# eboigne/PyTV-4D

Measured on NVIDIA B200. Metric: cp_iter_voxel_updates_per_s, higher is better.
Workload: dtype f32

## Files before the change

### pytv-4d_b200/csrc/adj_core.cuh

```cuda
#pragma once
#include "strip_core.cuh"

#ifndef PYTVB_STRIP_R
#define PYTVB_STRIP_R 4
#endif
#ifndef PYTVB_ADJ_R
#define PYTVB_ADJ_R 32
#endif

namespace pytvb {

constexpr int ADJ_R = PYTVB_ADJ_R;
constexpr int ADJ_MAXM = 8;
constexpr int ADJ_THREADS = 256;
static_assert(ADJ_R % PYTVB_STRIP_R == 0, "the L21 partial sums follow the row groups of cp_dual_strip_kernel");

PYTVB_HD int adj_tile_quads(int M) { return M == 1 ? 256 : (M == 2 ? 128 : (M <= 4 ? 64 : 32)); }

PYTVB_HD bool adj_edge_row(int i, int Ni) { return (i % ADJ_R == 0 && i > 0) || (i % ADJ_R == ADJ_R - 1 && i < Ni - 1); }
PYTVB_HD bool adj_edge_col(int tq, int TWq, int j0, int vec, int Nj) { return (tq == 0 && j0 > 0) || (tq == TWq - 1 && j0 + vec < Nj); }

template <int VEC> struct AdjSlots { static constexpr int value = 3 + 2 * VEC; };
template <typename T, int VEC>
struct AdjShared {
    T* b;
    PYTVB_HD T& jf0(int k) const { return b[k]; }
    PYTVB_HD T& jf1(int k) const { return b[ADJ_THREADS + k]; }
    PYTVB_HD T& jb0(int k) const { return b[2 * ADJ_THREADS + k]; }
    PYTVB_HD T& tf(int e, int k) const { return b[(3 + e) * ADJ_THREADS + k]; }
    PYTVB_HD T& tb(int e, int k) const { return b[(3 + VEC + e) * ADJ_THREADS + k]; }
};

template <typename T, int VEC, int SCHEME, bool Z_ON, bool T_ON>
struct AdjThread {
    static constexpr int ND = Comp<SCHEME, Z_ON, T_ON>::ND;
    DualPlane<T, T> pl;
    MirrorPlanes<T> mir;
    T* qp;
    int t, tq, j0, TWq;
    bool act, cedge;
    T at, bt;
    T yv[ND][VEC], tsc[VEC];
    T cIFm[VEC], cIF[VEC], cIB[VEC], cCol[VEC], cT[VEC];
    T g;
    double l21;
};

template <typename T, int VEC, int SCHEME, bool Z_ON, bool T_ON, bool MIR>
PYTVB_HD void adj_thread_init(AdjThread<T, VEC, SCHEME, Z_ON, T_ON>& s, const ImgView<T>& Xb, T* y, T* qd, const Params<T>& P, const MirrorBufs<T>& mb,
                              int z, int cb, int tid, int TWq, int W) {
    s.TWq = TWq;
    s.t = tid / TWq;
    s.tq = tid - s.t * TWq;
    const int qj = cb * TWq + s.tq;
    s.j0 = qj * VEC;
    s.act = s.t < P.M && qj < W;
    const int tc = s.t < P.M ? s.t : P.M - 1;
    s.pl = make_dual_plane<T, SCHEME, T>(Xb, y, P, z, tc);
    s.mir = MirrorPlanes<T>{nullptr, nullptr};
    if constexpr (MIR) s.mir = mirror_planes<T>(mb, P, z, tc);
    s.qp = qd + (long long)z * P.sZ + (long long)tc * P.sT;
    s.cedge = adj_edge_col(s.tq, TWq, s.j0, VEC, P.Nj);
    s.at = s.bt = T(0);
    if (T_ON) {
        adj_factors<T, SCHEME>(s.at, s.bt, tc, P.M, P.t_fwd_fallback != 0);
        s.at *= P.srt;
        s.bt *= P.srt;
    }
#pragma unroll
    for (int e = 0; e < VEC; ++e) s.cIFm[e] = s.cIF[e] = s.cIB[e] = s.cCol[e] = s.cT[e] = T(0);
    s.g = T(0);
    s.l21 = 0.0;
}

template <typename T, int VEC, int SCHEME, bool Z_ON, bool T_ON>
PYTVB_HD void adj_finish_row(AdjThread<T, VEC, SCHEME, Z_ON, T_ON>& s, const Params<T>& P, int k, const T* ib_next) {
    constexpr bool NF = (SCHEME != DOWNWIND), NB = (SCHEME != UPWIND), CTR = (SCHEME == CENTRAL);
    T a, b;
    adj_factors<T, SCHEME>(a, b, k, P.Ni, false);
    Pack<T, VEC> pk;
#pragma unroll
    for (int e = 0; e < VEC; ++e) {
        const T f_m = NF ? (k > 0 ? s.cIFm[e] : s.cIF[e]) : T(0);
        const T f_c = (!CTR && NF) ? s.cIF[e] : T(0);
        const T b_c = (!CTR && NB) ? s.cIB[e] : T(0);
        const T b_p = NB ? ib_next[e] : T(0);
        const T rows = adj_term<T, SCHEME>(a, b, f_m, f_c, b_c, b_p, false);
        pk.v[e] = s.cedge ? adj_rows_t<T, T_ON>(rows, s.cT[e]) : adj_prefix<T, T_ON>(rows, s.cCol[e], s.cT[e]);
    }
    if (!adj_edge_row(k, P.Ni)) st_pack<T, VEC>(s.qp + k * P.Nj + s.j0, pk);
}

template <typename T, int VEC, int SCHEME, bool Z_ON, bool T_ON>
PYTVB_HD void adj_prefetch_next(const AdjThread<T, VEC, SCHEME, Z_ON, T_ON>& s, const Params<T>& P, int i) {
#if defined(__CUDA_ARCH__)
    const int Nj = P.Nj, o = i * Nj + s.j0;
#pragma unroll
    for (int k = 0; k < Comp<SCHEME, Z_ON, T_ON>::ND; ++k) asm volatile("prefetch.global.L2 [%0];" ::"l"(s.pl.y + (long long)k * P.sC + o + Nj));
    asm volatile("prefetch.global.L2 [%0];" ::"l"(s.pl.c + (i + 2 < P.Ni ? o + 2 * Nj : o + Nj)));
#else
    (void)s; (void)P; (void)i;
#endif
}

template <typename T, int VEC, int SCHEME, bool Z_ON, bool T_ON, bool TS, bool MIR>
PYTVB_HD void adj_row_update(AdjThread<T, VEC, SCHEME, Z_ON, T_ON>& s, const Params<T>& P, int i, const AdjShared<T, VEC>& sh, int tid, T sig, T lam) {
    typedef Comp<SCHEME, Z_ON, T_ON> C;
    if (!s.act) return;
    const int Nj = P.Nj, o = i * Nj + s.j0;
    s.g += strip_quad_cp_dual_y<T, VEC, SCHEME, Z_ON, T_ON, T, TS, MIR>(s.yv, s.pl, P, i, s.j0, o, i > 0 ? o - Nj : o, i < P.Ni - 1 ? o + Nj : o, sig,
                                                                       lam, s.mir);
    if (i % PYTVB_STRIP_R == PYTVB_STRIP_R - 1 || i == P.Ni - 1) {
        s.l21 += (double)s.g * (double)P.inv_div;
        s.g = T(0);
    }
    sh.jf0(tid) = s.yv[C::J_F][0];
    sh.jf1(tid) = s.yv[C::J_F][VEC - 1];
    sh.jb0(tid) = s.yv[C::J_B][0];
    if (T_ON) {
#pragma unroll
        for (int e = 0; e < VEC; ++e) s.tsc[e] = T(1);
        if constexpr (TS) {
            const Pack<T, VEC> sc = ld_pack<T, VEC>(s.pl.ts + o);
#pragma unroll
            for (int e = 0; e < VEC; ++e) s.tsc[e] = sc.v[e];
        }
#pragma unroll
        for (int e = 0; e < VEC; ++e) {
            sh.tf(e, tid) = TS ? mul_rn(s.yv[C::T_F][e], s.tsc[e]) : s.yv[C::T_F][e];
            sh.tb(e, tid) = TS ? mul_rn(s.yv[C::T_B][e], s.tsc[e]) : s.yv[C::T_B][e];
        }
    }
}

template <typename T, int VEC, int SCHEME, bool Z_ON, bool T_ON, bool TS>
PYTVB_HD void adj_row_finish(AdjThread<T, VEC, SCHEME, Z_ON, T_ON>& s, const Params<T>& P, int i, bool first, const AdjShared<T, VEC>& sh, int tid) {
    typedef Comp<SCHEME, Z_ON, T_ON> C;
    constexpr bool NF = (SCHEME != DOWNWIND), NB = (SCHEME != UPWIND), CTR = (SCHEME == CENTRAL);
    constexpr bool HB = (SCHEME == HYBRID || SCHEME == DOWNWIND);
    if (!s.act) return;
    const int Nj = P.Nj, TWq = s.TWq;
    T col[VEC], tt[VEC];
    {
        T jb[VEC];
#pragma unroll
        for (int e = 0; e < VEC; ++e) jb[e] = (SCHEME == HYBRID) ? s.yv[C::J_B][e] : T(0);
        const bool has_l = s.j0 > 0 && s.tq > 0, has_r = s.j0 + VEC < Nj && s.tq < TWq - 1;
        const T jf_l = (NF && has_l) ? sh.jf1(tid - 1) : T(0);
        const T jf_r = (CTR && has_r) ? sh.jf0(tid + 1) : T(0);
        const T jb_r = (HB && has_r) ? sh.jb0(tid + 1) : T(0);
        adj_cols<T, VEC, SCHEME>(col, s.yv[C::J_F], jb, jf_l, jf_r, jb_r, s.j0, Nj);
    }
    if (T_ON) {
        const bool tfb = P.t_fwd_fallback != 0, up_form = !CTR || tfb;
        T ifs[VEC], f_m[VEC], f_c[VEC], b_c[VEC], b_p[VEC], fac[VEC];
#pragma unroll
        for (int e = 0; e < VEC; ++e) {
            ifs[e] = TS ? mul_rn(s.yv[C::I_F][e], s.tsc[e]) : s.yv[C::I_F][e];
            f_m[e] = NF ? (s.t > 0 ? sh.tf(e, tid - TWq) : ifs[e]) : T(0);
            f_c[e] = (up_form && NF) ? sh.tf(e, tid) : T(0);
            b_c[e] = (!CTR && NB) ? sh.tb(e, tid) : T(0);
            b_p[e] = (NB && !(CTR && tfb)) ? (s.t < P.M - 1 ? sh.tb(e, tid + TWq) : ifs[e]) : T(0);
        }
        static_factor<T, VEC>(fac, P, i, s.j0);
        adj_time<T, VEC, SCHEME>(tt, f_m, f_c, b_c, b_p, fac, s.at, s.bt, tfb);
    } else {
        zero_into<T, VEC>(tt);
    }
    if (!first) adj_finish_row(s, P, i - 1, s.yv[C::I_B]);
#pragma unroll
    for (int e = 0; e < VEC; ++e) {
        s.cIFm[e] = s.cIF[e];
        s.cIF[e] = s.yv[C::I_F][e];
        s.cIB[e] = s.yv[C::I_B][e];
        s.cCol[e] = col[e];
        s.cT[e] = tt[e];
    }
}

template <typename T, int VEC, int SCHEME, bool Z_ON, bool T_ON>
PYTVB_HD void adj_tile_end(AdjThread<T, VEC, SCHEME, Z_ON, T_ON>& s, const Params<T>& P, int i_end) {
    if (s.act && i_end == P.Ni) adj_finish_row(s, P, P.Ni - 1, s.cIB);
}

template <typename T, int VEC, int SCHEME, bool Z_ON, bool T_ON, int VARIANT, bool WM, bool TS, bool MIR>
PYTVB_HD T adj_quad_primal(const PrimalPlane<T, T>& pl, const T* qd, T* x, T* xbar, const T* x0, const T* w, const Params<T>& P, int i, int j0,
                           bool cedge, T tau, T c1, T theta, T tau_x0, MirrorPlanes<T> mir) {
    typedef Comp<SCHEME, Z_ON, T_ON> C;
    constexpr bool NF = (SCHEME != DOWNWIND), CTR = (SCHEME == CENTRAL), HB = (SCHEME == HYBRID || SCHEME == DOWNWIND);
    const int o = i * P.Nj + j0;
    T dty[VEC];
    if (adj_edge_row(i, P.Ni)) {
        strip_quad_DT<T, VEC, SCHEME, Z_ON, T_ON, false, T, TS>(dty, pl, P, i, j0, o, i > 0 ? o - P.Nj : o, i < P.Ni - 1 ? o + P.Nj : o);
    } else {
        const T* qo = qd + pl.img + o;
        const T* yJ_F = pl.y + (long long)C::J_F * P.sC + o;
        const T* yJ_B = pl.y + (long long)C::J_B * P.sC + o;
        const bool l = cedge && NF && j0 > 0, rf = cedge && CTR && j0 + VEC < P.Nj, rb = cedge && HB && j0 + VEC < P.Nj;
        T jf[VEC], jb[VEC];
        ld_into<T, VEC>(jf, cedge ? yJ_F : qo);
        if (SCHEME == HYBRID) ld_into<T, VEC>(jb, cedge ? yJ_B : qo); else zero_into<T, VEC>(jb);
        T jf_l = *(l ? yJ_F - 1 : qo), jf_r = *(rf ? yJ_F + VEC : qo), jb_r = *(rb ? yJ_B + VEC : qo);
        jf_l = l ? jf_l : T(0); jf_r = rf ? jf_r : T(0); jb_r = rb ? jb_r : T(0);
        const Pack<T, VEC> pre = ld_pack<T, VEC>(qo);
        T zt[VEC], cols[VEC];
        if (Z_ON) strip_quad_DT_z<T, VEC, SCHEME, Z_ON, T_ON, false, T>(zt, pl, P, o); else zero_into<T, VEC>(zt);
        adj_cols<T, VEC, SCHEME>(cols, jf, jb, jf_l, jf_r, jb_r, j0, P.Nj);
#pragma unroll
        for (int e = 0; e < VEC; ++e) dty[e] = adj_finish<T, Z_ON>(cedge ? add_rn(pre.v[e], cols[e]) : pre.v[e], zt[e], P.inv_div);
    }
    return cp_primal_update<T, VEC, Z_ON, VARIANT, MIR, WM>(dty, x, xbar, x0, pl.img + o, o, tau, c1, theta, tau_x0, mir, w);
}

}
```

### pytv-4d_b200/csrc/cp_adj.cu

```cuda
#include <stdlib.h>

#include "host_common.cuh"
#include "kernels2.cuh"
#include "adj_core.cuh"

using namespace pytvb;

namespace pytvb {

static_assert(ADJ_THREADS == CTA_THREADS, "an A' tile is one CTA");

struct AdjTiling {
    int TWq, W, ncb, nz;
    FastDiv d_ncb, d_nz;
    long long nblocks;
};
inline AdjTiling make_adj_tiling(int Nj, int Ni, int M, int nz, int vec) {
    AdjTiling t;
    t.TWq = adj_tile_quads(M);
    t.W = (Nj + vec - 1) / vec;
    t.ncb = (t.W + t.TWq - 1) / t.TWq;
    t.nz = nz;
    t.d_ncb = make_fastdiv((unsigned)t.ncb);
    t.d_nz = make_fastdiv((unsigned)nz);
    t.nblocks = (long long)t.ncb * nz * ((Ni + ADJ_R - 1) / ADJ_R);
    return t;
}

template <typename T, int VEC, int SCHEME, bool Z_ON, bool T_ON, bool TS, bool MIR>
__global__ void __launch_bounds__(CTA_THREADS, PYTVB_DUAL_MINB) cp_dual_adj_kernel(ImgView<T> Xb, T* __restrict__ y, T* __restrict__ qd,
                                                                                  double* __restrict__ partial, Params<T> P, T sig, T lam,
                                                                                  AdjTiling tl, MirrorBufs<T> mb) {
    __shared__ T sm[2][AdjSlots<T_ON ? VEC : 0>::value * CTA_THREADS];
    unsigned b = blockIdx.x, cb, zi;
    tl.d_ncb.divmod(b, b, cb);
    tl.d_nz.divmod(b, b, zi);
    const int i0 = (int)b * ADJ_R, nrows = min(ADJ_R, P.Ni - i0), tid = threadIdx.x;
    AdjThread<T, VEC, SCHEME, Z_ON, T_ON> s;
    adj_thread_init<T, VEC, SCHEME, Z_ON, T_ON, MIR>(s, Xb, y, qd, P, mb, (int)zi, (int)cb, tid, tl.TWq, tl.W);
    for (int r = 0; r < nrows; ++r) {
        const int bf = r & 1;
        const AdjShared<T, VEC> sh{sm[bf]};
        if (s.act && r + 1 < nrows) adj_prefetch_next(s, P, i0 + r);
        adj_row_update<T, VEC, SCHEME, Z_ON, T_ON, TS, MIR>(s, P, i0 + r, sh, tid, sig, lam);
        __syncthreads();
        adj_row_finish<T, VEC, SCHEME, Z_ON, T_ON, TS>(s, P, i0 + r, r == 0, sh, tid);
    }
    adj_tile_end(s, P, i0 + nrows);
    if (partial) {
        const double bs = block_sum(s.l21);
        store_or_finish(bs, partial, P);
    }
}

template <typename T, int VEC, int SCHEME, bool Z_ON, bool T_ON, int VARIANT, bool WM, int R, bool TS, bool MIR>
__global__ void __launch_bounds__(CTA_THREADS, PYTVB_PRIMAL_MINB) cp_primal_adj_kernel(FieldView<T> Y, const T* __restrict__ qd, T* __restrict__ x,
                                                                                      T* __restrict__ xbar, const T* __restrict__ x0,
                                                                                      const T* __restrict__ w, double* __restrict__ partial,
                                                                                      Params<T> P, T tau, T c1, T theta, T tau_x0, Tiling tl,
                                                                                      int twq, MirrorBufs<T> mb) {
    const QuadIdx q = decode_quad(tl, (P.Ni + R - 1) / R, VEC);
    T fid = T(0);
    if (q.active) {
        const PrimalPlane<T, T> pl = make_primal_plane<T, SCHEME, Z_ON, T_ON, T>(Y, P, q.z, q.t);
        MirrorPlanes<T> mir{nullptr, nullptr};
        if constexpr (MIR) mir = mirror_planes<T>(mb, P, q.z, q.t);
        const bool cedge = adj_edge_col((q.j0 / VEC) & (twq - 1), twq, q.j0, VEC, P.Nj);
        const int i0 = q.i * R;
#pragma unroll
        for (int r = 0; r < R; ++r) {
            const int i = i0 + r;
            if (i < P.Ni)
                fid += adj_quad_primal<T, VEC, SCHEME, Z_ON, T_ON, VARIANT, WM, TS, MIR>(pl, qd, x, xbar, x0, w, P, i, q.j0, cedge, tau, c1, theta, tau_x0,
                                                                                         mir);
        }
    }
    if (partial) {
        const double bs = block_sum((double)fid);
        store_or_finish(bs, partial, P);
    }
}

}

namespace {

template <typename T> struct AdjDualArgs { ImgView<T> Xb; T* y; T* q; double* partial; Params<T> P; T sig, lam; cudaStream_t st; long long* nb; T* mir_prev; T* mir_next; };

template <typename T, int VEC, int SCHEME, bool Z, bool TT> struct LaunchDualAdj {
    static int run(const AdjDualArgs<T>& a) {
        const AdjTiling tl = make_adj_tiling(a.P.Nj, a.P.Ni, a.P.M, a.P.Nz, VEC);
        PYTVB_REQUIRE(tl.nblocks > 0 && tl.nblocks < 2147483647LL, "grid of %lld CTAs is out of range", tl.nblocks);
        const bool ts = TT && a.P.tscale, mir = Z && (a.mir_prev || a.mir_next);
        const MirrorBufs<T> mb{a.mir_prev, a.mir_next};
        const unsigned nb = (unsigned)tl.nblocks;
        if (ts && mir) cp_dual_adj_kernel<T, VEC, SCHEME, Z, TT, TT, Z><<<nb, CTA_THREADS, 0, a.st>>>(a.Xb, a.y, a.q, a.partial, a.P, a.sig, a.lam, tl, mb);
        else if (ts) cp_dual_adj_kernel<T, VEC, SCHEME, Z, TT, TT, false><<<nb, CTA_THREADS, 0, a.st>>>(a.Xb, a.y, a.q, a.partial, a.P, a.sig, a.lam, tl, mb);
        else if (mir) cp_dual_adj_kernel<T, VEC, SCHEME, Z, TT, false, Z><<<nb, CTA_THREADS, 0, a.st>>>(a.Xb, a.y, a.q, a.partial, a.P, a.sig, a.lam, tl, mb);
        else cp_dual_adj_kernel<T, VEC, SCHEME, Z, TT, false, false><<<nb, CTA_THREADS, 0, a.st>>>(a.Xb, a.y, a.q, a.partial, a.P, a.sig, a.lam, tl, mb);
        count_launches(1);
        PYTVB_CUDA(cudaGetLastError());
        *a.nb = tl.nblocks;
        return PYTVB_OK;
    }
};

template <typename T> struct AdjPrimalArgs {
    FieldView<T> Y; const T* q; T* x; T* xbar; const T* x0; const T* w; double* partial; Params<T> P; T tau, theta; int term; cudaStream_t st;
    long long* nb; T* mir_prev; T* mir_next;
};

template <typename T, int VEC, int SCHEME, bool Z, bool TT, int VARIANT, bool WM>
void launch_primal_adj(const AdjPrimalArgs<T>& a, const Tiling& tl) {
    constexpr int R = PYTVB_STRIP_R;
    const bool ts = TT && a.P.tscale, mir = Z && (a.mir_prev || a.mir_next);
    const MirrorBufs<T> mb{a.mir_prev, a.mir_next};
    const unsigned nb = (unsigned)tl.nblocks;
    const T c1 = VARIANT == 0 ? T(1) / (T(1) + a.tau) : T(0), tx = VARIANT == 0 ? T(-1) : a.tau;
    const int twq = adj_tile_quads(a.P.M);
#define PYTVB_ADJ_B(TSV, MIRV)                                                                                                                  \
    cp_primal_adj_kernel<T, VEC, SCHEME, Z, TT, VARIANT, WM, R, TSV, MIRV><<<nb, CTA_THREADS, 0, a.st>>>(a.Y, a.q, a.x, a.xbar, a.x0, a.w, a.partial, \
                                                                                                      a.P, a.tau, c1, a.theta, tx, tl, twq, mb)
    if (ts && mir) PYTVB_ADJ_B(TT, Z);
    else if (ts) PYTVB_ADJ_B(TT, false);
    else if (mir) PYTVB_ADJ_B(false, Z);
    else PYTVB_ADJ_B(false, false);
#undef PYTVB_ADJ_B
}

template <typename T, int VEC, int SCHEME, bool Z, bool TT> struct LaunchPrimalAdj {
    static int run(const AdjPrimalArgs<T>& a) {
        const Tiling tl = make_strip_tiling<PYTVB_STRIP_R>(a.P.Nj, a.P.Ni, a.P.M, a.P.Nz, VEC);
        if (int rc = check_grid(tl)) return rc;
        if (a.term == PYTVB_DATA_L2 && !a.w) launch_primal_adj<T, VEC, SCHEME, Z, TT, 0, false>(a, tl);
        else if (a.term == PYTVB_DATA_L2) launch_primal_adj<T, VEC, SCHEME, Z, TT, 2, true>(a, tl);
        else if (a.w) launch_primal_adj<T, VEC, SCHEME, Z, TT, 3, true>(a, tl);
        else launch_primal_adj<T, VEC, SCHEME, Z, TT, 3, false>(a, tl);
        count_launches(1);
        PYTVB_CUDA(cudaGetLastError());
        *a.nb = tl.nblocks;
        return PYTVB_OK;
    }
};

template <typename T>
int run_dual_adj(const pytvb_problem* pb, const void* xbar, void* y, void* q, double lam, double sigma, double* d_l21, const void* lo, const void* hi,
                 void* mir_prev, void* mir_next, void* ws, cudaStream_t st) {
    const Axes ax = axes_of(pb);
    AdjDualArgs<T> a;
    a.Xb = ImgView<T>{(const T*)xbar, (const T*)lo, (const T*)hi, 1};
    a.y = (T*)y;
    a.q = (T*)q;
    a.partial = d_l21 ? reduce_partials(ws) : nullptr;
    a.P = make_params<T>(pb);
    arm_reduction(a.P, ws, d_l21);
    a.sig = (T)sigma * a.P.inv_div;
    a.lam = (T)lam;
    a.mir_prev = (T*)mir_prev; a.mir_next = (T*)mir_next;
    a.st = st;
    long long nb = 0;
    a.nb = &nb;
    const int vec = pick_vec<T>(pb, {xbar, y, q, lo, hi, mir_prev, mir_next});
    if (int rc = dispatch<LaunchDualAdj, T>(vec, pb->scheme, ax.z_on, ax.t_on, a)) return rc;
    return d_l21 ? finish_reduction(a.partial, nb, d_l21, st) : PYTVB_OK;
}

template <typename T>
int run_primal_adj(const pytvb_problem* pb, int term, const void* w, const void* y, const void* q, void* x, void* xbar, const void* x0, double tau,
                   double theta, double* d_fid, const void* lo, const void* hi, void* mir_prev, void* mir_next, void* ws, cudaStream_t st) {
    const Axes ax = axes_of(pb);
    AdjPrimalArgs<T> a;
    a.Y = FieldView<T>{(const T*)y, (const T*)lo, (const T*)hi};
    a.q = (const T*)q;
    a.x = (T*)x; a.xbar = (T*)xbar; a.x0 = (const T*)x0; a.w = (const T*)w;
    a.partial = d_fid ? reduce_partials(ws) : nullptr;
    a.P = make_params<T>(pb);
    arm_reduction(a.P, ws, d_fid);
    a.tau = (T)tau; a.theta = (T)theta;
    a.term = term;
    a.mir_prev = (T*)mir_prev; a.mir_next = (T*)mir_next;
    a.st = st;
    long long nb = 0;
    a.nb = &nb;
    const int vec = pick_vec<T>(pb, {y, q, x, xbar, x0, w, lo, hi, mir_prev, mir_next});
    if (int rc = dispatch<LaunchPrimalAdj, T>(vec, pb->scheme, ax.z_on, ax.t_on, a)) return rc;
    return d_fid ? finish_reduction(a.partial, nb, d_fid, st) : PYTVB_OK;
}

}

extern "C" {

int pytvb_cp_dual_adj_p2p(const pytvb_problem* pb, const void* xbar, void* y, void* q, double lam, double sigma, double* d_l21_or_null,
                          const void* halo_lo, const void* halo_hi, void* mirror_prev, void* mirror_next, void* ws, void* stream) {
    if (int rc = check_problem(pb)) return rc;
    PYTVB_REQUIRE(xbar && y && q, "xbar, y and q must not be NULL");
    PYTVB_REQUIRE(pb->M <= ADJ_MAXM, "M = %lld: the dual pass with the adjoint prefix spans at most %d frames", (long long)pb->M, ADJ_MAXM);
    PYTVB_REQUIRE(!d_l21_or_null || ws, "a reduction workspace is required when d_l21 is requested");
    PYTVB_REQUIRE(lam >= 0, "lam must be >= 0");
    if (int rc = check_halos(pb, axes_of(pb).z_on, false, halo_lo, halo_hi)) return rc;
    cudaStream_t st = (cudaStream_t)stream;
    return pb->dtype == PYTVB_F32 ? run_dual_adj<float>(pb, xbar, y, q, lam, sigma, d_l21_or_null, halo_lo, halo_hi, mirror_prev, mirror_next, ws, st)
                                  : run_dual_adj<double>(pb, xbar, y, q, lam, sigma, d_l21_or_null, halo_lo, halo_hi, mirror_prev, mirror_next, ws, st);
}

int pytvb_cp_dual_adj(const pytvb_problem* pb, const void* xbar, void* y, void* q, double lam, double sigma, double* d_l21_or_null, const void* halo_lo,
                      const void* halo_hi, void* ws, void* stream) {
    return pytvb_cp_dual_adj_p2p(pb, xbar, y, q, lam, sigma, d_l21_or_null, halo_lo, halo_hi, nullptr, nullptr, ws, stream);
}

int pytvb_cp_primal_adj_p2p(const pytvb_problem* pb, int data_term, const void* data_weight, const void* y, const void* q, void* x, void* xbar,
                            const void* x0, double tau, double theta, double* d_fid_or_null, const void* halo_lo, const void* halo_hi,
                            void* mirror_prev, void* mirror_next, void* ws, void* stream) {
    if (int rc = check_problem(pb)) return rc;
    PYTVB_REQUIRE(data_term == PYTVB_DATA_L2 || data_term == PYTVB_DATA_L1, "data_term must be PYTVB_DATA_L2 (0) or PYTVB_DATA_L1 (1)");
    PYTVB_REQUIRE(y && q && x && xbar && x0, "y, q, x, xbar and x0 must not be NULL");
    PYTVB_REQUIRE(pb->M <= ADJ_MAXM, "M = %lld: the dual pass with the adjoint prefix spans at most %d frames", (long long)pb->M, ADJ_MAXM);
    PYTVB_REQUIRE(!d_fid_or_null || ws, "a reduction workspace is required when d_fid is requested");
    if (int rc = check_halos(pb, axes_of(pb).z_on, true, halo_lo, halo_hi)) return rc;
    cudaStream_t st = (cudaStream_t)stream;
    return pb->dtype == PYTVB_F32 ? run_primal_adj<float>(pb, data_term, data_weight, y, q, x, xbar, x0, tau, theta, d_fid_or_null, halo_lo, halo_hi,
                                                          mirror_prev, mirror_next, ws, st)
                                  : run_primal_adj<double>(pb, data_term, data_weight, y, q, x, xbar, x0, tau, theta, d_fid_or_null, halo_lo, halo_hi,
                                                           mirror_prev, mirror_next, ws, st);
}

int pytvb_cp_primal_adj(const pytvb_problem* pb, int data_term, const void* data_weight, const void* y, const void* q, void* x, void* xbar,
                        const void* x0, double tau, double theta, double* d_fid_or_null, const void* halo_lo, const void* halo_hi, void* ws,
// ... 7 lines not shown
```

### pytv-4d_b200/csrc/strip_core.cuh

```cuda
#pragma once
#include <cuda_fp16.h>

#include "core.cuh"

namespace pytvb {

PYTVB_HD float fast_rsqrt(float a) {
#if defined(__CUDA_ARCH__)
    return rsqrtf(a);
#else
    return 1.0f / sqrtf(a);
#endif
}
PYTVB_HD double fast_rsqrt(double a) { return 1.0 / sqrt(a); }
PYTVB_HD float fast_sqrt(float a) {
#if defined(__CUDA_ARCH__)
    float r;
    asm("sqrt.approx.f32 %0, %1;" : "=f"(r) : "f"(a));
    return r;
#else
    return sqrtf(a);
#endif
}
PYTVB_HD double fast_sqrt(double a) { return sqrt(a); }
// ... 330 lines not shown
PYTVB_HD void adj_cols(T* out, const T* jf, const T* jb, T jf_left, T jf_right, T jb_right, int j0, int Nj) {
    T f[VEC + 2], bq[VEC + 2];
    f[0] = jf_left;
#pragma unroll
    for (int e = 0; e < VEC; ++e) f[e + 1] = jf[e];
    f[VEC + 1] = jf_right;
#pragma unroll
    for (int e = 0; e < VEC + 2; ++e) bq[e] = (SCHEME == DOWNWIND) ? f[e] : T(0);
    if (SCHEME == HYBRID) {
#pragma unroll
        for (int e = 0; e < VEC; ++e) bq[e + 1] = jb[e];
    }
    if (SCHEME == HYBRID || SCHEME == DOWNWIND) bq[VEC + 1] = jb_right;
#pragma unroll
    for (int e = 0; e < VEC; ++e) {
        T a, b;
        adj_factors<T, SCHEME>(a, b, j0 + e, Nj, false);
        out[e] = (SCHEME == CENTRAL) ? adj_term<T, SCHEME>(a, b, f[e], T(0), T(0), f[e + 2], false)
                                     : adj_term<T, SCHEME>(a, b, f[e], f[e + 1], bq[e + 1], bq[e + 2], false);
    }
}

template <typename T, bool T_ON>
PYTVB_HD T adj_rows_t(T rows, T t) {
    return T_ON ? add_rn(rows, t) : rows;
}
template <typename T, bool T_ON>
PYTVB_HD T adj_prefix(T rows, T cols, T t) {
    return add_rn(adj_rows_t<T, T_ON>(rows, t), cols);
}
template <typename T, bool Z_ON>
PYTVB_HD T adj_finish(T prefix, T z, T inv_div) {
    return mul_rn(Z_ON ? add_rn(prefix, z) : prefix, inv_div);
}

template <typename T, int VEC> struct CgLoad;
#if defined(__CUDACC__)
template <> struct CgLoad<float, 4> { static __device__ __forceinline__ void ld(float* d, const float* p) { const float4 v = __ldcg(reinterpret_cast<const float4*>(p)); d[0] = v.x; d[1] = v.y; d[2] = v.z; d[3] = v.w; } };
template <> struct CgLoad<float, 1> { static __device__ __forceinline__ void ld(float* d, const float* p) { d[0] = __ldcg(p); } };
template <> struct CgLoad<double, 2> { static __device__ __forceinline__ void ld(double* d, const double* p) { const double2 v = __ldcg(reinterpret_cast<const double2*>(p)); d[0] = v.x; d[1] = v.y; } };
template <> struct CgLoad<double, 1> { static __device__ __forceinline__ void ld(double* d, const double* p) { d[0] = __ldcg(p); } };
#endif
template <typename T, int VEC, bool CG, typename YT>
PYTVB_HD void ld_field(T* dst, const YT* src) {
#if defined(__CUDA_ARCH__)
    if constexpr (CG) { CgLoad<T, VEC>::ld(dst, (const T*)src); return; }
#endif
    ld_y<T, YT, VEC>(dst, src);
}
template <typename T, bool CG, typename YT>
PYTVB_HD T ld_field1(const YT* src) {
#if defined(__CUDA_ARCH__)
    if constexpr (CG) { T v; CgLoad<T, 1>::ld(&v, (const T*)src); return v; }
#endif
    T v;
    ld_y<T, YT, 1>(&v, src);
    return v;
}

template <typename T, int VEC>
PYTVB_HD void scale_by_rn(T* v, const T* ts_plane, int o) {
    if (ts_plane) {
        const Pack<T, VEC> sc = ld_pack<T, VEC>(ts_plane + o);
#pragma unroll
        for (int e = 0; e < VEC; ++e) v[e] = mul_rn(v[e], sc.v[e]);
    }
}

template <typename T, int VEC, int SCHEME>
PYTVB_HD void adj_time(T* out, const T* f_m, const T* f_c, const T* b_c, const T* b_p, const T* fac, T at, T bt, bool fb) {
#pragma unroll
    for (int e = 0; e < VEC; ++e) out[e] = mul_rn(adj_term<T, SCHEME>(at, bt, f_m[e], f_c[e], b_c[e], b_p[e], fb), fac[e]);
}

template <typename T, int VEC, int SCHEME, bool Z_ON, bool T_ON, bool CG, typename YT, bool TS>
PYTVB_HD void strip_quad_DT_prefix(T* pre, const PrimalPlane<T, YT>& pl, const Params<T>& P, int i, int j0, int o, int o_up, int o_dn) {
    typedef Comp<SCHEME, Z_ON, T_ON> C;
    constexpr bool NF = (SCHEME != DOWNWIND);
    constexpr bool NB = (SCHEME != UPWIND);
    constexpr bool CTR = (SCHEME == CENTRAL);
    const YT* yI_F = pl.y + (long long)C::I_F * P.sC;
    const YT* yI_B = pl.y + (long long)C::I_B * P.sC;
    const YT* yJ_F = pl.y + (long long)C::J_F * P.sC;
    const YT* yJ_B = pl.y + (long long)C::J_B * P.sC;
    T rows[VEC], cols[VEC], tt[VEC];
    {
        T a, b, f_m[VEC], f_c[VEC], b_c[VEC], b_p[VEC];
        adj_factors<T, SCHEME>(a, b, i, P.Ni, false);
        if (NF) ld_field<T, VEC, CG>(f_m, yI_F + o_up); else zero_into<T, VEC>(f_m);
        if (!CTR && NF) ld_field<T, VEC, CG>(f_c, yI_F + o); else zero_into<T, VEC>(f_c);
        if (!CTR && NB) ld_field<T, VEC, CG>(b_c, yI_B + o); else zero_into<T, VEC>(b_c);
        if (NB) ld_field<T, VEC, CG>(b_p, yI_B + o_dn); else zero_into<T, VEC>(b_p);
#pragma unroll
        for (int e = 0; e < VEC; ++e) rows[e] = adj_term<T, SCHEME>(a, b, f_m[e], f_c[e], b_c[e], b_p[e], false);
    }
    {
        T jf[VEC], jb[VEC];
        ld_field<T, VEC, CG>(jf, yJ_F + o);
        if (SCHEME == HYBRID) ld_field<T, VEC, CG>(jb, yJ_B + o); else zero_into<T, VEC>(jb);
        const T jf_l = (NF && j0 > 0) ? ld_field1<T, CG>(yJ_F + o - 1) : T(0);
        const T jf_r = (CTR && j0 + VEC < P.Nj) ? ld_field1<T, CG>(yJ_F + o + VEC) : T(0);
        const T jb_r = ((SCHEME == HYBRID || SCHEME == DOWNWIND) && j0 + VEC < P.Nj) ? ld_field1<T, CG>(yJ_B + o + VEC) : T(0);
        adj_cols<T, VEC, SCHEME>(cols, jf, jb, jf_l, jf_r, jb_r, j0, P.Nj);
    }
    if (T_ON) {
        const bool fb = P.t_fwd_fallback != 0;
        const bool up_form = !CTR || fb;
        T f_m[VEC], f_c[VEC], b_c[VEC], b_p[VEC], fac[VEC];
        if (NF) ld_field<T, VEC, CG>(f_m, pl.tf_m + o); else zero_into<T, VEC>(f_m);
        if (up_form && NF) ld_field<T, VEC, CG>(f_c, pl.y + (long long)C::T_F * P.sC + o); else zero_into<T, VEC>(f_c);
        if (!CTR && NB) ld_field<T, VEC, CG>(b_c, pl.y + (long long)C::T_B * P.sC + o); else zero_into<T, VEC>(b_c);
        if (NB && !(CTR && fb)) ld_field<T, VEC, CG>(b_p, pl.tb_p + o); else zero_into<T, VEC>(b_p);
        if constexpr (TS) {
            scale_by_rn<T, VEC>(f_m, pl.ts_m, o); scale_by_rn<T, VEC>(f_c, pl.ts_c, o);
            scale_by_rn<T, VEC>(b_c, pl.ts_c, o); scale_by_rn<T, VEC>(b_p, pl.ts_p, o);
        }
        static_factor<T, VEC>(fac, P, i, j0);
        adj_time<T, VEC, SCHEME>(tt, f_m, f_c, b_c, b_p, fac, pl.at, pl.bt, fb);
    }
#pragma unroll
    for (int e = 0; e < VEC; ++e) pre[e] = adj_prefix<T, T_ON>(rows[e], cols[e], T_ON ? tt[e] : T(0));
}

template <typename T, int VEC, int SCHEME, bool Z_ON, bool T_ON, bool CG, typename YT>
PYTVB_HD void strip_quad_DT_z(T* zt, const PrimalPlane<T, YT>& pl, const Params<T>& P, int o) {
    typedef Comp<SCHEME, Z_ON, T_ON> C;
    constexpr bool NF = (SCHEME != DOWNWIND), NB = (SCHEME != UPWIND), CTR = (SCHEME == CENTRAL);
    const bool fb = P.z_fwd_fallback != 0;
    const bool up_form = !CTR || fb;
    T f_m[VEC], f_c[VEC], b_c[VEC], b_p[VEC];
    if (NF) ld_field<T, VEC, CG>(f_m, pl.zf_m + o); else zero_into<T, VEC>(f_m);
    if (up_form && NF) ld_field<T, VEC, CG>(f_c, pl.y + (long long)C::Z_F * P.sC + o); else zero_into<T, VEC>(f_c);
    if (!CTR && NB) ld_field<T, VEC, CG>(b_c, pl.y + (long long)C::Z_B * P.sC + o); else zero_into<T, VEC>(b_c);
    if (NB && !(CTR && fb)) ld_field<T, VEC, CG>(b_p, pl.zb_p + o); else zero_into<T, VEC>(b_p);
#pragma unroll
    for (int e = 0; e < VEC; ++e) zt[e] = adj_term<T, SCHEME>(pl.az, pl.bz, f_m[e], f_c[e], b_c[e], b_p[e], fb);
}

template <typename T, int VEC, int SCHEME, bool Z_ON, bool T_ON, bool CG, typename YT, bool TS>
PYTVB_HD void strip_quad_DT_impl(T* out, const PrimalPlane<T, YT>& pl, const Params<T>& P, int i, int j0, int o, int o_up, int o_dn) {
    T pre[VEC], zt[VEC];
    strip_quad_DT_prefix<T, VEC, SCHEME, Z_ON, T_ON, CG, YT, TS>(pre, pl, P, i, j0, o, o_up, o_dn);
    if (Z_ON) strip_quad_DT_z<T, VEC, SCHEME, Z_ON, T_ON, CG, YT>(zt, pl, P, o); else zero_into<T, VEC>(zt);
#pragma unroll
    for (int e = 0; e < VEC; ++e) out[e] = adj_finish<T, Z_ON>(pre[e], zt[e], P.inv_div);
}

template <typename T, int VEC, int SCHEME, bool Z_ON, bool T_ON, bool CG = false, typename YT = T, bool TS = false>
PYTVB_HD void strip_quad_DT(T* out, const PrimalPlane<T, YT>& pl, const Params<T>& P, int i, int j0, int o, int o_up, int o_dn) {
    strip_quad_DT_impl<T, VEC, SCHEME, Z_ON, T_ON, CG, YT, TS && T_ON>(out, pl, P, i, j0, o, o_up, o_dn);
}

template <typename T, int VEC, bool Z_ON, int VARIANT, bool MIR, bool WM>
PYTVB_HD T cp_primal_update(const T* dty, T* x, T* aux, const T* x0, long long off, int o, T tau, T c1, T c2, T tau_x0, MirrorPlanes<T> mir,
                            const T* wgt) {
    if (tau_x0 < T(0)) tau_x0 = tau;
    const Pack<T, VEC> xo = ld_pack<T, VEC>(x + off), x0q = ld_pack<T, VEC>(x0 + off);
    Pack<T, VEC> xn, ax;
    T fid = T(0);
    if constexpr (VARIANT == 0) {
#pragma unroll
        for (int e = 0; e < VEC; ++e) {
            xn.v[e] = (xo.v[e] - tau * dty[e] + tau_x0 * x0q.v[e]) * c1;
            ax.v[e] = xn.v[e] + c2 * (xn.v[e] - xo.v[e]);
            const T r = xn.v[e] - x0q.v[e];
            fid += r * r;
        }
    } else if constexpr (VARIANT == 1) {
        const Pack<T, VEC> yf = ld_pack<T, VEC>(aux + off);
#pragma unroll
        for (int e = 0; e < VEC; ++e) {
            ax.v[e] = (yf.v[e] + c2 * (xo.v[e] - x0q.v[e])) * c1;
            xn.v[e] = xo.v[e] - tau * ax.v[e] - tau * dty[e];
            const T r = xn.v[e] - x0q.v[e];
            fid += r * r;
        }
    } else {
        static_assert(VARIANT == 2 || VARIANT == 3, "unknown primal variant");
        Pack<T, VEC> wq;
        if constexpr (WM) wq = ld_pack<T, VEC>(wgt + off);
#pragma unroll
        for (int e = 0; e < VEC; ++e) {
            T w = T(1), tw = tau_x0;
            if constexpr (WM) { w = wq.v[e]; tw = tau_x0 * w; }
            const T v = xo.v[e] - tau * dty[e];
            T r;
            if constexpr (VARIANT == 2) {
                xn.v[e] = (v + tw * x0q.v[e]) / (T(1) + tw);
                r = xn.v[e] - x0q.v[e];
                fid += w * (r * r);
            } else {
                const T d = v - x0q.v[e];
                const T a = (d < T(0) ? -d : d) - tw;
                const T s = a > T(0) ? a : T(0);
                xn.v[e] = x0q.v[e] + (d < T(0) ? -s : s);
                r = xn.v[e] - x0q.v[e];
                fid += w * (r < T(0) ? -r : r);
            }
            ax.v[e] = xn.v[e] + c2 * (xn.v[e] - xo.v[e]);
        }
    }
    st_pack<T, VEC>(x + off, xn);
    st_pack<T, VEC>(aux + off, ax);
    if constexpr (MIR && Z_ON) {
        const Pack<T, VEC>& u = (VARIANT == 1) ? xn : ax;
        if (mir.prev) st_pack<T, VEC>(mir.prev + o, u);
        if (mir.next) st_pack<T, VEC>(mir.next + o, u);
    }
    return fid;
}

template <typename T, int VEC, int SCHEME, bool Z_ON, bool T_ON, int VARIANT, bool CG = false, typename YT = T, bool TS = false, bool MIR = false,
          bool WM = false>
PYTVB_HD T strip_quad_cp_primal(T* x, T* aux, const T* x0, const PrimalPlane<T, YT>& pl, const Params<T>& P, int i, int j0, int o, int o_up, int o_dn,
                                T tau, T c1, T c2, T tau_x0 = T(-1), MirrorPlanes<T> mir = MirrorPlanes<T>{nullptr, nullptr}, const T* wgt = nullptr) {
    T dty[VEC];
    strip_quad_DT<T, VEC, SCHEME, Z_ON, T_ON, CG, YT, TS>(dty, pl, P, i, j0, o, o_up, o_dn);
    return cp_primal_update<T, VEC, Z_ON, VARIANT, MIR, WM>(dty, x, aux, x0, pl.img + o, o, tau, c1, c2, tau_x0, mir, wgt);
}

template <typename T>
struct GradPlane {
    const T* x;  const T* xzm;  const T* xzp;  const T* xtm;  const T* xtp;
    const T* xzm2; const T* xzp2; const T* xtm2; const T* xtp2;
    const T* w;  const T* wzm;  const T* wzp;  const T* wtm;  const T* wtp;
    T az, bz, at, bt;
    bool z_fb, t_fb;
    const T* ts_m; const T* ts_c; const T* ts_p;
};

template <typename T, int SCHEME>
PYTVB_HD GradPlane<T> make_grad_plane(const ImgView<T>& X, const ImgView<T>& W, const Params<T>& P, int z, int t) {
    GradPlane<T> g;
    const long long zg = P.zg0 + z;
    const bool v_zm = zg > 0, v_zp = zg < P.NzG - 1, v_tm = t > 0, v_tp = t < P.M - 1;
    g.x = X.row(P, z, t, 0);
    g.w = W.row(P, z, t, 0);
    g.xzm = v_zm ? X.row(P, z - 1, t, 0) : g.x;  g.wzm = v_zm ? W.row(P, z - 1, t, 0) : g.w;
    g.xzp = v_zp ? X.row(P, z + 1, t, 0) : g.x;  g.wzp = v_zp ? W.row(P, z + 1, t, 0) : g.w;
    g.xtm = v_tm ? X.row(P, z, t - 1, 0) : g.x;  g.wtm = v_tm ? W.row(P, z, t - 1, 0) : g.w;
    g.xtp = v_tp ? X.row(P, z, t + 1, 0) : g.x;  g.wtp = v_tp ? W.row(P, z, t + 1, 0) : g.w;
    g.xzm2 = g.xzp2 = g.xtm2 = g.xtp2 = g.x;
    g.az = g.bz = P.srz;
    g.at = g.bt = P.srt;
    g.z_fb = P.z_fwd_fallback != 0;
    g.t_fb = P.t_fwd_fallback != 0;
    g.ts_m = g.ts_c = g.ts_p = nullptr;
    if (P.tscale) {
        g.ts_c = P.tscale + (long long)z * P.sZ + (long long)t * P.sT;
        g.ts_m = v_tm ? g.ts_c - P.sT : g.ts_c;
        g.ts_p = v_tp ? g.ts_c + P.sT : g.ts_c;
    }
    if (SCHEME == CENTRAL) {
        if (!g.z_fb) {
            if (zg >= 2) g.xzm2 = X.row(P, z - 2, t, 0); else g.az = T(0);
            if (zg <= P.NzG - 3) g.xzp2 = X.row(P, z + 2, t, 0); else g.bz = T(0);
        }
        if (!g.t_fb) {
            if (t >= 2) g.xtm2 = X.row(P, z, t - 2, 0); else g.at = T(0);
            if (t <= P.M - 3) g.xtp2 = X.row(P, z, t + 2, 0); else g.bt = T(0);
        }
    }
    return g;
}

template <typename T, int SCHEME>
PYTVB_HD T strip_g_axis(bool fallback, T a, T b, T xm2, T xm, T xc, T xp, T xp2, T wm, T wc, T wp) {
    if (SCHEME == UPWIND || (SCHEME == CENTRAL && fallback)) return (xc - xm) * wm - (xp - xc) * wc;
    if (SCHEME == DOWNWIND) return (xc - xm) * wc - (xp - xc) * wp;
    if (SCHEME == HYBRID) return (xc - xm) * (wm + wc) - (xp - xc) * (wc + wp);
    return a * ((xc - xm2) * wm) - b * ((xp2 - xc) * wp);
}

template <typename T, int VEC, int SCHEME, bool Z_ON, bool T_ON, bool TS, bool ROWS = true>
PYTVB_HD void strip_quad_G_impl(T* g_plane, const GradPlane<T>& pl, const Params<T>& P, int i, int j0, int o, const T* g_rows = nullptr) {
    constexpr bool CEN = (SCHEME == CENTRAL);
    const int Nj = P.Nj;
    const int o_up = i > 0 ? o - Nj : o, o_dn = i < P.Ni - 1 ? o + Nj : o;
    T xr[VEC + 4], wr[VEC + 2];
    ld_into<T, VEC>(xr + 2, pl.x + o);
    ld_into<T, VEC>(wr + 1, pl.w + o);
    xr[1] = j0 > 0 ? pl.x[o - 1] : xr[2];
    wr[0] = j0 > 0 ? pl.w[o - 1] : wr[1];
    xr[VEC + 2] = j0 + VEC < Nj ? pl.x[o + VEC] : xr[VEC + 1];
    wr[VEC + 1] = j0 + VEC < Nj ? pl.w[o + VEC] : wr[VEC];
    xr[0] = (CEN && j0 > 1) ? pl.x[o - 2] : xr[1];
    xr[VEC + 3] = (CEN && j0 + VEC + 1 < Nj) ? pl.x[o + VEC + 1] : xr[VEC + 2];
    T g[VEC];
#pragma unroll
    for (int e = 0; e < VEC; ++e) {
        const int j = j0 + e;
        const T a = (CEN && j < 2) ? T(0) : T(1), b = (CEN && j > Nj - 3) ? T(0) : T(1);
        g[e] = strip_g_axis<T, SCHEME>(false, a, b, xr[e], xr[e + 1], xr[e + 2], xr[e + 3], xr[e + 4], wr[e], wr[e + 1], wr[e + 2]);
    }
    if constexpr (ROWS) {
        T xm[VEC], xp[VEC], wm[VEC], wp[VEC], xm2[VEC], xp2[VEC];
        ld_into<T, VEC>(xm, pl.x + o_up);  ld_into<T, VEC>(xp, pl.x + o_dn);
        ld_into<T, VEC>(wm, pl.w + o_up);  ld_into<T, VEC>(wp, pl.w + o_dn);
        T a = T(1), b = T(1);
        if (CEN) {
            ld_into<T, VEC>(xm2, pl.x + (i > 1 ? o - 2 * Nj : o));
            ld_into<T, VEC>(xp2, pl.x + (i < P.Ni - 2 ? o + 2 * Nj : o));
            a = i >= 2 ? T(1) : T(0);
            b = i <= P.Ni - 3 ? T(1) : T(0);
        }
#pragma unroll
        for (int e = 0; e < VEC; ++e)
            g[e] += strip_g_axis<T, SCHEME>(false, a, b, CEN ? xm2[e] : T(0), xm[e], xr[e + 2], xp[e], CEN ? xp2[e] : T(0), wm[e], wr[e + 1], wp[e]);
    } else {
#pragma unroll
        for (int e = 0; e < VEC; ++e) g[e] += g_rows[e];
    }
    if (Z_ON) {
        T xm[VEC], xp[VEC], wm[VEC], wp[VEC], xm2[VEC], xp2[VEC];
        ld_into<T, VEC>(xm, pl.xzm + o);  ld_into<T, VEC>(xp, pl.xzp + o);
        ld_into<T, VEC>(wm, pl.wzm + o);  ld_into<T, VEC>(wp, pl.wzp + o);
        if (CEN) { ld_into<T, VEC>(xm2, pl.xzm2 + o); ld_into<T, VEC>(xp2, pl.xzp2 + o); }
#pragma unroll
        for (int e = 0; e < VEC; ++e) {
            const T v = strip_g_axis<T, SCHEME>(pl.z_fb, pl.az, pl.bz, CEN ? xm2[e] : T(0), xm[e], xr[e + 2], xp[e], CEN ? xp2[e] : T(0), wm[e], wr[e + 1], wp[e]);
            g[e] += (CEN && !pl.z_fb) ? v : P.srz * v;
        }
    }
    if (T_ON) {
        T xm[VEC], xp[VEC], wm[VEC], wp[VEC], xm2[VEC], xp2[VEC], fac[VEC];
        ld_into<T, VEC>(xm, pl.xtm + o);  ld_into<T, VEC>(xp, pl.xtp + o);
        ld_into<T, VEC>(wm, pl.wtm + o);  ld_into<T, VEC>(wp, pl.wtp + o);
        if (CEN) { ld_into<T, VEC>(xm2, pl.xtm2 + o); ld_into<T, VEC>(xp2, pl.xtp2 + o); }
        static_factor<T, VEC>(fac, P, i, j0);
        T wc[VEC];
#pragma unroll
        for (int e = 0; e < VEC; ++e) wc[e] = wr[e + 1];
        if constexpr (TS) {
            scale_by<T, VEC>(wm, pl.ts_m, o); scale_by<T, VEC>(wc, pl.ts_c, o); scale_by<T, VEC>(wp, pl.ts_p, o);
        }
#pragma unroll
        for (int e = 0; e < VEC; ++e) {
            const T v = strip_g_axis<T, SCHEME>(pl.t_fb, pl.at, pl.bt, CEN ? xm2[e] : T(0), xm[e], xr[e + 2], xp[e], CEN ? xp2[e] : T(0), wm[e], wc[e], wp[e]);
            g[e] += ((CEN && !pl.t_fb) ? v : P.srt * v) * fac[e];
        }
    }
    Pack<T, VEC> pk;
#pragma unroll
    for (int e = 0; e < VEC; ++e) pk.v[e] = g[e] * (P.inv_div * P.inv_div);
    st_pack<T, VEC>(g_plane + o, pk);
}

template <typename T, int VEC, int SCHEME, bool Z_ON, bool T_ON, bool TS = false>
PYTVB_HD void strip_quad_G(T* g_plane, const GradPlane<T>& pl, const Params<T>& P, int i, int j0, int o) {
    strip_quad_G_impl<T, VEC, SCHEME, Z_ON, T_ON, TS && T_ON>(g_plane, pl, P, i, j0, o);
}


template <typename T, int SCHEME>
PYTVB_HD T pair_w(T wk, T wk1) {
    return SCHEME == UPWIND ? wk : (SCHEME == DOWNWIND ? wk1 : wk + wk1);
}

template <typename T>
PYTVB_HD void row_neighbours(T& l, T& r, const T* row_o, T first, T last, bool has_l, bool has_r, int vec, bool wrow, unsigned m,
                             bool need_l, bool need_r) {
#if defined(__CUDA_ARCH__)
// ... 373 lines not shown
```

Measured before the change: 60.01 billion.

## Double adjoint row tile height and add L2 prefetch of primal rows

Raises the default adjoint dual tile height from 32 to 64 rows, which halves the halo and edge-row overhead per tile. It also adds an L2 prefetch pass over all R rows of qd, z-components, x, x0 and weights before the primal adjoint loop, which is on by default (BMODE 2). A batched-load primal path and a configurable prefetch distance are added behind macros that are off by default. Taller tiles mean fewer CTAs and may reduce parallelism on small grids, and the extra prefetch instructions add issue overhead.

```diff
diff --git a/pytv-4d_b200/csrc/adj_core.cuh b/pytv-4d_b200/csrc/adj_core.cuh
--- a/pytv-4d_b200/csrc/adj_core.cuh
+++ b/pytv-4d_b200/csrc/adj_core.cuh
@@ -5,7 +5,7 @@
 #define PYTVB_STRIP_R 4
 #endif
 #ifndef PYTVB_ADJ_R
-#define PYTVB_ADJ_R 32
+#define PYTVB_ADJ_R 64
 #endif
 
 namespace pytvb {
@@ -92,12 +92,12 @@
 }
 
 template <typename T, int VEC, int SCHEME, bool Z_ON, bool T_ON>
-PYTVB_HD void adj_prefetch_next(const AdjThread<T, VEC, SCHEME, Z_ON, T_ON>& s, const Params<T>& P, int i) {
+PYTVB_HD void adj_prefetch_next(const AdjThread<T, VEC, SCHEME, Z_ON, T_ON>& s, const Params<T>& P, int i, int d = 1) {
 #if defined(__CUDA_ARCH__)
     const int Nj = P.Nj, o = i * Nj + s.j0;
 #pragma unroll
-    for (int k = 0; k < Comp<SCHEME, Z_ON, T_ON>::ND; ++k) asm volatile("prefetch.global.L2 [%0];" ::"l"(s.pl.y + (long long)k * P.sC + o + Nj));
-    asm volatile("prefetch.global.L2 [%0];" ::"l"(s.pl.c + (i + 2 < P.Ni ? o + 2 * Nj : o + Nj)));
+    for (int k = 0; k < Comp<SCHEME, Z_ON, T_ON>::ND; ++k) asm volatile("prefetch.global.L2 [%0];" ::"l"(s.pl.y + (long long)k * P.sC + o + d * Nj));
+    asm volatile("prefetch.global.L2 [%0];" ::"l"(s.pl.c + (i + d + 1 < P.Ni ? o + (d + 1) * Nj : o + d * Nj)));
 #else
     (void)s; (void)P; (void)i;
 #endif
@@ -183,33 +183,90 @@
     if (s.act && i_end == P.Ni) adj_finish_row(s, P, P.Ni - 1, s.cIB);
 }
 
+template <typename T, int VEC, int SCHEME, bool Z_ON, bool T_ON>
+PYTVB_HD void adj_quad_dty(T* dty, const PrimalPlane<T, T>& pl, const T* qo, const Params<T>& P, int o, int j0, bool cedge) {
+    typedef Comp<SCHEME, Z_ON, T_ON> C;
+    constexpr bool NF = (SCHEME != DOWNWIND), CTR = (SCHEME == CENTRAL), HB = (SCHEME == HYBRID || SCHEME == DOWNWIND);
+    const T* yJ_F = pl.y + (long long)C::J_F * P.sC + o;
+    const T* yJ_B = pl.y + (long long)C::J_B * P.sC + o;
+    const bool l = cedge && NF && j0 > 0, rf = cedge && CTR && j0 + VEC < P.Nj, rb = cedge && HB && j0 + VEC < P.Nj;
+    T jf[VEC], jb[VEC];
+    ld_into<T, VEC>(jf, cedge ? yJ_F : qo);
+    if (SCHEME == HYBRID) ld_into<T, VEC>(jb, cedge ? yJ_B : qo); else zero_into<T, VEC>(jb);
+    T jf_l = *(l ? yJ_F - 1 : qo), jf_r = *(rf ? yJ_F + VEC : qo), jb_r = *(rb ? yJ_B + VEC : qo);
+    jf_l = l ? jf_l : T(0); jf_r = rf ? jf_r : T(0); jb_r = rb ? jb_r : T(0);
+    const Pack<T, VEC> pre = ld_pack<T, VEC>(qo);
+    T zt[VEC], cols[VEC];
+    if (Z_ON) strip_quad_DT_z<T, VEC, SCHEME, Z_ON, T_ON, false, T>(zt, pl, P, o); else zero_into<T, VEC>(zt);
+    adj_cols<T, VEC, SCHEME>(cols, jf, jb, jf_l, jf_r, jb_r, j0, P.Nj);
+#pragma unroll
+    for (int e = 0; e < VEC; ++e) dty[e] = adj_finish<T, Z_ON>(cedge ? add_rn(pre.v[e], cols[e]) : pre.v[e], zt[e], P.inv_div);
+}
+
 template <typename T, int VEC, int SCHEME, bool Z_ON, bool T_ON, int VARIANT, bool WM, bool TS, bool MIR>
 PYTVB_HD T adj_quad_primal(const PrimalPlane<T, T>& pl, const T* qd, T* x, T* xbar, const T* x0, const T* w, const Params<T>& P, int i, int j0,
                            bool cedge, T tau, T c1, T theta, T tau_x0, MirrorPlanes<T> mir) {
-    typedef Comp<SCHEME, Z_ON, T_ON> C;
-    constexpr bool NF = (SCHEME != DOWNWIND), CTR = (SCHEME == CENTRAL), HB = (SCHEME == HYBRID || SCHEME == DOWNWIND);
     const int o = i * P.Nj + j0;
     T dty[VEC];
-    if (adj_edge_row(i, P.Ni)) {
+    if (adj_edge_row(i, P.Ni))
         strip_quad_DT<T, VEC, SCHEME, Z_ON, T_ON, false, T, TS>(dty, pl, P, i, j0, o, i > 0 ? o - P.Nj : o, i < P.Ni - 1 ? o + P.Nj : o);
-    } else {
-        const T* qo = qd + pl.img + o;
-        const T* yJ_F = pl.y + (long long)C::J_F * P.sC + o;
-        const T* yJ_B = pl.y + (long long)C::J_B * P.sC + o;
-        const bool l = cedge && NF && j0 > 0, rf = cedge && CTR && j0 + VEC < P.Nj, rb = cedge && HB && j0 + VEC < P.Nj;
-        T jf[VEC], jb[VEC];
-        ld_into<T, VEC>(jf, cedge ? yJ_F : qo);
-        if (SCHEME == HYBRID) ld_into<T, VEC>(jb, cedge ? yJ_B : qo); else zero_into<T, VEC>(jb);
-        T jf_l = *(l ? yJ_F - 1 : qo), jf_r = *(rf ? yJ_F + VEC : qo), jb_r = *(rb ? yJ_B + VEC : qo);
-        jf_l = l ? jf_l : T(0); jf_r = rf ? jf_r : T(0); jb_r = rb ? jb_r : T(0);
-        const Pack<T, VEC> pre = ld_pack<T, VEC>(qo);
-        T zt[VEC], cols[VEC];
-        if (Z_ON) strip_quad_DT_z<T, VEC, SCHEME, Z_ON, T_ON, false, T>(zt, pl, P, o); else zero_into<T, VEC>(zt);
-        adj_cols<T, VEC, SCHEME>(cols, jf, jb, jf_l, jf_r, jb_r, j0, P.Nj);
-#pragma unroll
-        for (int e = 0; e < VEC; ++e) dty[e] = adj_finish<T, Z_ON>(cedge ? add_rn(pre.v[e], cols[e]) : pre.v[e], zt[e], P.inv_div);
-    }
+    else
+        adj_quad_dty<T, VEC, SCHEME, Z_ON, T_ON>(dty, pl, qd + pl.img + o, P, o, j0, cedge);
     return cp_primal_update<T, VEC, Z_ON, VARIANT, MIR, WM>(dty, x, xbar, x0, pl.img + o, o, tau, c1, theta, tau_x0, mir, w);
 }
 
-}
+template <typename T, int VEC, int SCHEME, bool Z_ON, bool T_ON, bool WM, int R>
+PYTVB_HD void adj_prefetch_rows(const PrimalPlane<T, T>& pl, const T* qd, const T* x, const T* x0, const T* w, const Params<T>& P, int i0, int j0) {
+#if defined(__CUDA_ARCH__)
+    typedef Comp<SCHEME, Z_ON, T_ON> C;
+#pragma unroll
+    for (int r = 0; r < R; ++r) {
+        const int i = i0 + r < P.Ni ? i0 + r : P.Ni - 1, o = i * P.Nj + j0;
+        const long long off = pl.img + o;
+        if (!adj_edge_row(i, P.Ni)) asm volatile("prefetch.global.L2 [%0];" ::"l"(qd + off));
+        if (Z_ON) {
+            asm volatile("prefetch.global.L2 [%0];" ::"l"(pl.y + (long long)C::Z_F * P.sC + o));
+            if (C::Z_B != C::Z_F) asm volatile("prefetch.global.L2 [%0];" ::"l"(pl.y + (long long)C::Z_B * P.sC + o));
+        }
+        asm volatile("prefetch.global.L2 [%0];" ::"l"(x + off));
+        asm volatile("prefetch.global.L2 [%0];" ::"l"(x0 + off));
+        if (WM) asm volatile("prefetch.global.L2 [%0];" ::"l"(w + off));
+    }
+#else
+    (void)pl; (void)qd; (void)x; (void)x0; (void)w; (void)P; (void)i0; (void)j0;
+#endif
+}
+
+template <typename T, int VEC, int SCHEME, bool Z_ON, bool T_ON, int VARIANT, bool WM, bool TS, bool MIR, int R, int RB>
+PYTVB_HD T adj_rows_primal(const PrimalPlane<T, T>& pl, const T* qd, T* x, T* xbar, const T* x0, const T* w, const Params<T>& P, int i0, int j0,
+                           bool cedge, T tau, T c1, T theta, T tau_x0, MirrorPlanes<T> mir) {
+    const int Nj = P.Nj;
+    T fid = T(0);
+#pragma unroll
+    for (int b = 0; b < R; b += RB) {
+        T dty[RB][VEC];
+        Pack<T, VEC> xo[RB], x0q[RB], wq[RB];
+#pragma unroll
+        for (int r = 0; r < RB; ++r) {
+            const int i = i0 + b + r < P.Ni ? i0 + b + r : P.Ni - 1, o = i * Nj + j0;
+            const long long off = pl.img + o;
+            adj_quad_dty<T, VEC, SCHEME, Z_ON, T_ON>(dty[r], pl, adj_edge_row(i, P.Ni) ? x + off : qd + off, P, o, j0, cedge);
+            xo[r] = ld_pack<T, VEC>(x + off);
+            x0q[r] = ld_pack<T, VEC>(x0 + off);
+            if constexpr (WM) wq[r] = ld_pack<T, VEC>(w + off);
+        }
+#pragma unroll
+        for (int r = 0; r < RB; ++r) {
+            const int i = i0 + b + r, o = i * Nj + j0;
+            if (i < P.Ni) {
+                if (adj_edge_row(i, P.Ni))
+                    strip_quad_DT<T, VEC, SCHEME, Z_ON, T_ON, false, T, TS>(dty[r], pl, P, i, j0, o, i > 0 ? o - Nj : o, i < P.Ni - 1 ? o + Nj : o);
+                fid += cp_primal_apply<T, VEC, Z_ON, VARIANT, MIR, WM>(dty[r], xo[r], x0q[r], wq[r], x, xbar, pl.img + o, o, tau, c1, theta, tau_x0,
+                                                                       mir);
+            }
+        }
+    }
+    return fid;
+}
+
+}
diff --git a/pytv-4d_b200/csrc/cp_adj.cu b/pytv-4d_b200/csrc/cp_adj.cu
--- a/pytv-4d_b200/csrc/cp_adj.cu
+++ b/pytv-4d_b200/csrc/cp_adj.cu
@@ -41,7 +41,11 @@
     for (int r = 0; r < nrows; ++r) {
         const int bf = r & 1;
         const AdjShared<T, VEC> sh{sm[bf]};
-        if (s.act && r + 1 < nrows) adj_prefetch_next(s, P, i0 + r);
+#ifndef PYTVB_ADJ_PFD
+#define PYTVB_ADJ_PFD 1
+#endif
+        if (PYTVB_ADJ_PFD == 2 && s.act && r == 0 && r + 1 < nrows) adj_prefetch_next(s, P, i0 + r, 1);
+        if (s.act && r + PYTVB_ADJ_PFD < nrows) adj_prefetch_next(s, P, i0 + r, PYTVB_ADJ_PFD);
         adj_row_update<T, VEC, SCHEME, Z_ON, T_ON, TS, MIR>(s, P, i0 + r, sh, tid, sig, lam);
         __syncthreads();
         adj_row_finish<T, VEC, SCHEME, Z_ON, T_ON, TS>(s, P, i0 + r, r == 0, sh, tid);
@@ -54,7 +58,16 @@
 }
 
 template <typename T, int VEC, int SCHEME, bool Z_ON, bool T_ON, int VARIANT, bool WM, int R, bool TS, bool MIR>
-__global__ void __launch_bounds__(CTA_THREADS, PYTVB_PRIMAL_MINB) cp_primal_adj_kernel(FieldView<T> Y, const T* __restrict__ qd, T* __restrict__ x,
+#ifndef PYTVB_ADJ_BMODE
+#define PYTVB_ADJ_BMODE 2
+#endif
+#ifndef PYTVB_ADJ_RB
+#define PYTVB_ADJ_RB 4
+#endif
+#ifndef PYTVB_ADJ_PMINB
+#define PYTVB_ADJ_PMINB PYTVB_PRIMAL_MINB
+#endif
+__global__ void __launch_bounds__(CTA_THREADS, PYTVB_ADJ_PMINB) cp_primal_adj_kernel(FieldView<T> Y, const T* __restrict__ qd, T* __restrict__ x,
                                                                                       T* __restrict__ xbar, const T* __restrict__ x0,
                                                                                       const T* __restrict__ w, double* __restrict__ partial,
                                                                                       Params<T> P, T tau, T c1, T theta, T tau_x0, Tiling tl,
@@ -66,7 +79,14 @@
         MirrorPlanes<T> mir{nullptr, nullptr};
         if constexpr (MIR) mir = mirror_planes<T>(mb, P, q.z, q.t);
         const bool cedge = adj_edge_col((q.j0 / VEC) & (twq - 1), twq, q.j0, VEC, P.Nj);
+#if PYTVB_ADJ_BMODE == 1
+        fid = adj_rows_primal<T, VEC, SCHEME, Z_ON, T_ON, VARIANT, WM, TS, MIR, R, PYTVB_ADJ_RB>(pl, qd, x, xbar, x0, w, P, q.i * R, q.j0, cedge, tau, c1, theta, tau_x0,
+                                                                                   mir);
+#else
         const int i0 = q.i * R;
+#if PYTVB_ADJ_BMODE == 2
+        adj_prefetch_rows<T, VEC, SCHEME, Z_ON, T_ON, WM, R>(pl, qd, x, x0, w, P, i0, q.j0);
+#endif
 #pragma unroll
         for (int r = 0; r < R; ++r) {
             const int i = i0 + r;
@@ -74,6 +94,7 @@
                 fid += adj_quad_primal<T, VEC, SCHEME, Z_ON, T_ON, VARIANT, WM, TS, MIR>(pl, qd, x, xbar, x0, w, P, i, q.j0, cedge, tau, c1, theta, tau_x0,
                                                                                          mir);
         }
+#endif
     }
     if (partial) {
         const double bs = block_sum((double)fid);
diff --git a/pytv-4d_b200/csrc/strip_core.cuh b/pytv-4d_b200/csrc/strip_core.cuh
--- a/pytv-4d_b200/csrc/strip_core.cuh
+++ b/pytv-4d_b200/csrc/strip_core.cuh
@@ -506,10 +506,9 @@
 }
 
 template <typename T, int VEC, bool Z_ON, int VARIANT, bool MIR, bool WM>
-PYTVB_HD T cp_primal_update(const T* dty, T* x, T* aux, const T* x0, long long off, int o, T tau, T c1, T c2, T tau_x0, MirrorPlanes<T> mir,
-                            const T* wgt) {
+PYTVB_HD T cp_primal_apply(const T* dty, const Pack<T, VEC>& xo, const Pack<T, VEC>& x0q, const Pack<T, VEC>& wq, T* x, T* aux, long long off, int o,
+                           T tau, T c1, T c2, T tau_x0, MirrorPlanes<T> mir) {
     if (tau_x0 < T(0)) tau_x0 = tau;
-    const Pack<T, VEC> xo = ld_pack<T, VEC>(x + off), x0q = ld_pack<T, VEC>(x0 + off);
     Pack<T, VEC> xn, ax;
     T fid = T(0);
     if constexpr (VARIANT == 0) {
@@ -531,8 +530,6 @@
         }
     } else {
         static_assert(VARIANT == 2 || VARIANT == 3, "unknown primal variant");
-        Pack<T, VEC> wq;
-        if constexpr (WM) wq = ld_pack<T, VEC>(wgt + off);
 #pragma unroll
         for (int e = 0; e < VEC; ++e) {
             T w = T(1), tw = tau_x0;
@@ -562,6 +559,14 @@
         if (mir.next) st_pack<T, VEC>(mir.next + o, u);
     }
     return fid;
+}
+template <typename T, int VEC, bool Z_ON, int VARIANT, bool MIR, bool WM>
+PYTVB_HD T cp_primal_update(const T* dty, T* x, T* aux, const T* x0, long long off, int o, T tau, T c1, T c2, T tau_x0, MirrorPlanes<T> mir,
+                            const T* wgt) {
+    const Pack<T, VEC> xo = ld_pack<T, VEC>(x + off), x0q = ld_pack<T, VEC>(x0 + off);
+    Pack<T, VEC> wq;
+    if constexpr (WM) wq = ld_pack<T, VEC>(wgt + off);
+    return cp_primal_apply<T, VEC, Z_ON, VARIANT, MIR, WM>(dty, xo, x0q, wq, x, aux, off, o, tau, c1, c2, tau_x0, mir);
 }
 
 template <typename T, int VEC, int SCHEME, bool Z_ON, bool T_ON, int VARIANT, bool CG = false, typename YT = T, bool TS = false, bool MIR = false,
```

Measured after the change: 57.68 billion, median of 6. 0.961x the previous value.
